# Chemical118/TREW

Hardware: AMD Instinct MI355X
Metric: Gbases/s scanned (short 5 32, 150 bp reads) (higher is better)
Workload: dtype u32

## Files before the change

include/trew_hip.h:

```cpp
#ifndef TREW_HIP_H
#define TREW_HIP_H

#include <stddef.h>
#include <stdint.h>

#ifdef __cplusplus
extern "C" {
#endif

#define TREW_HIP_ABI_VERSION 4

enum {
    TREW_MODE_SHORT = 0,
    TREW_MODE_PAIR = 1,
    TREW_MODE_LONG = 2,
    TREW_MODE_SEGMENT = 3
};

enum {
    TREW_TABLE_FORWARD_HIGH = 0,
    TREW_TABLE_FORWARD_LOW = 1,
    TREW_TABLE_BACKWARD_HIGH = 2,
    TREW_TABLE_BACKWARD_LOW = 3,
    TREW_TABLE_BOTH_HIGH = 4,
    TREW_TABLE_BOTH_LOW = 5,
    TREW_NUM_TABLES = 6
};

enum {
    TREW_FLAG_NO_FILTER = 1,
    TREW_FLAG_DEBUG_NO_EMIT = 2,
    TREW_FLAG_DEBUG_NO_KLOOP = 4,
    TREW_FLAG_DEBUG_POISON_LDS = 32,
    TREW_FLAG_DEBUG_WIDE_NO_WAIT = 128,
    TREW_FLAG_NO_TIMING = 64,
    TREW_FLAG_COMPAT_G1 = 512,
    TREW_FLAG_DEBUG_NO_JOINT = 2048,
    TREW_FLAG_DEBUG_NO_UNI_DRAIN = 4096,
    TREW_FLAG_DEBUG_NO_GROUP = 1024,
    TREW_FLAG_DEBUG_ANNOT_GENERAL = 8192,
    TREW_FLAG_TRACK_PRESSURE = 256
};

typedef struct {
    int32_t min_mer;
    int32_t max_mer;
    double low_baseline;
    double high_baseline;
    int32_t slice_length;
    int32_t mode;
    int32_t device;
    int32_t n_slots;
    uint64_t max_batch_words;
    uint64_t max_batch_reads;
    uint32_t table_log2_slots;
    uint32_t flags;
    uint64_t max_batch_ascii_bytes;
} trew_hip_params;

typedef struct {
    const uint32_t *words;
    uint64_t n_words;
    const uint32_t *offsets;
    const uint32_t *lengths;
    uint32_t uniform_length;
    uint32_t uniform_stride;
    uint64_t n_reads;
    int32_t on_device;
    int32_t max_length;
} trew_hip_batch;

// ... 106 lines not shown
```

trew_amd/__init__.py:

```python
from . import capi
from .capi import (
    FLAG_NO_FILTER,
    FLAG_DEBUG_ANNOT_GENERAL,
    FLAG_DEBUG_POISON_LDS,
    FLAG_NO_TIMING,
    FLAG_TRACK_PRESSURE,
    FLAG_COMPAT_G1,
    FLAG_DEBUG_NO_GROUP,
    FLAG_DEBUG_NO_JOINT,
    FLAG_DEBUG_NO_UNI_DRAIN,
    FLAG_DEBUG_WIDE_NO_WAIT,
    MODE_LONG,
    MODE_PAIR,
    MODE_SEGMENT,
    MODE_SHORT,
    TABLE_NAMES,
    TrewHip,
    TrewHipError,
    annotate,
    k_mer_check,
    pack_reads,
)
```

trew_amd/capi.py:

```python
from __future__ import annotations

import ctypes as C
import os

import numpy as np

_HERE = os.path.dirname(os.path.abspath(__file__))
LIB_PATH = os.environ.get("TREW_HIP_LIB") or os.path.join(_HERE, "lib", "libtrew_hip.so")

MODE_SHORT, MODE_PAIR, MODE_LONG, MODE_SEGMENT = 0, 1, 2, 3
FLAG_NO_FILTER = 1
FLAG_DEBUG_POISON_LDS = 32
FLAG_NO_TIMING = 64
FLAG_COMPAT_G1 = 512
FLAG_TRACK_PRESSURE = 256
FLAG_DEBUG_NO_JOINT = 2048
FLAG_DEBUG_NO_UNI_DRAIN = 4096
FLAG_DEBUG_NO_GROUP = 1024
FLAG_DEBUG_ANNOT_GENERAL = 8192
FLAG_DEBUG_WIDE_NO_WAIT = 128
TABLE_NAMES = ("forward_high", "forward_low", "backward_high", "backward_low", "both_high", "both_low")

EXPORTED_SYMBOLS = (
    "trew_hip_init", "trew_hip_destroy", "trew_hip_last_error", "trew_hip_submit", "trew_hip_wait",
    "trew_hip_collect", "trew_hip_reset_tables", "trew_hip_add_rows", "trew_hip_segment_results",
    "trew_hip_filter_masks", "trew_hip_last_timing", "trew_pack_words", "trew_pack_reads",
    "trew_synth_short_ascii", "trew_synth_short_device", "trew_synth_pair_ascii", "trew_synth_pair_device",
    "trew_hip_malloc", "trew_hip_free", "trew_hip_memcpy_h2d", "trew_hip_memcpy_d2h", "trew_hip_abi_version",
    "trew_pack_pairs", "trew_hip_host_alloc", "trew_hip_host_free", "trew_hip_device_count",
    "trew_synth_long_lengths", "trew_synth_long_ascii", "trew_synth_long_device",
    "trew_hip_collect_device", "trew_hip_add_rows_device", "trew_hip_merge", "trew_hip_table_pressure",
    "trew_hip_add_gathered_device", "trew_hip_collect_slice_device", "trew_hip_debug_counters", "trew_hip_debug_worklist", "trew_hip_submit_ascii", "trew_hip_pack_ascii",
    "trew_motif_parse", "trew_hip_annotate", "trew_hip_annotate_results", "trew_annotate_host",
)
DEBUG_COUNTERS = ("strict_rerun", "windows_fallback", "wide_spin_timeout", "inserted", "inserted_wide", "group_punt", "group_routed", "group_target")


class Params(C.Structure):
    _fields_ = [
        ("min_mer", C.c_int32), ("max_mer", C.c_int32),
        ("low_baseline", C.c_double), ("high_baseline", C.c_double),
        ("slice_length", C.c_int32), ("mode", C.c_int32), ("device", C.c_int32), ("n_slots", C.c_int32),
        ("max_batch_words", C.c_uint64), ("max_batch_reads", C.c_uint64),
        ("table_log2_slots", C.c_uint32), ("flags", C.c_uint32),
        ("max_batch_ascii_bytes", C.c_uint64),
    ]


class Batch(C.Structure):
    _fields_ = [
# ... 473 lines not shown
```

trew_amd/csrc/kernels/decide_group.inc:

```

#define TREW_REGION_LIST(X) \
    X(chunk) X(stage) X(group_setup) X(bounds) X(group) X(dg_loop) X(dg_pick) X(dg_eval) X(er_gaps) X(er_runs) X(er_canon) X(er_merge) X(er_max) \
    X(dg_decision) X(dg_end) X(routing) X(records) X(target) X(target_rows) X(target_eval) X(target_emit) X(fallback)
#define TREW_REGION_ENUM(n) kRegion_##n,
enum { TREW_REGION_LIST(TREW_REGION_ENUM) kRegionCount };
#ifdef TREW_REGION_COUNTS
__device__ unsigned long long g_region[64];
#define TREW_MARK(n)                                                                   \
    do {                                                                               \
        asm volatile("; MARK " #n);                                                    \
        if (lane_id() == 0) atomicAdd(&g_region[kRegion_##n], 1ull);                   \
    } while (0)
#else
#define TREW_MARK(n) asm volatile("; MARK " #n)
#endif
__device__ __forceinline__ void lds_sync() {
    __builtin_amdgcn_fence(__ATOMIC_RELEASE, "wavefront");
    __builtin_amdgcn_wave_barrier();
    __builtin_amdgcn_fence(__ATOMIC_ACQUIRE, "wavefront");
}
#define TREW_DPP(v, ctrl) ((u32) __builtin_amdgcn_update_dpp(0, (int) (v), (ctrl), 0xf, 0xf, false))
__device__ __forceinline__ u32 swap16(u32 v) { return (u32) __builtin_amdgcn_ds_swizzle((int) v, 0x401F); }
template <int G = 16>
__device__ __forceinline__ u32 row_or(u32 v) {
// ... 242 lines not shown
    }
}

template <int NW>
struct RowSeg {
    u32 lo[NW], hi[NW], v1[NW], P1[NW], P2[NW], P3[NW];
    u32 has_n;
};
template <int NW, int G = 16>
__device__ __forceinline__ void row_load(ExactSmem sm, int L, RowSeg<NW> &r) {
    const u32 g = lane_id() / (u32) G;
    const u32 *prep = sm_group(sm) + kGroupBnd + g * (6u * NW);
    u32 anyn = 0;
#pragma unroll
    for (int w = 0; w < NW; w++) {
        r.lo[w] = prep[0 * NW + w];
        r.hi[w] = prep[1 * NW + w];
        r.v1[w] = prep[2 * NW + w];
        r.P1[w] = prep[3 * NW + w];
        r.P2[w] = prep[4 * NW + w];
        r.P3[w] = prep[5 * NW + w];
        const int bits = L - 32 * w;
        const u32 lm = bits >= 32 ? 0xffffffffu : (bits <= 0 ? 0u : ((1u << bits) - 1u));
        anyn |= ~r.v1[w] & lm;
    }
    r.has_n = anyn != 0u ? 1u : 0u;
}

template <int NW, bool SMALLK>
__device__ __forceinline__ u32 shr_k_word(const u32 (&x)[NW], int w, u32 k) {
    if (SMALLK) return alignbit(w + 1 < NW ? x[w + 1 < NW ? w + 1 : 0] : 0u, x[w], k);
    return shr_var_word<NW>(x, w, k);
}
template <int NW, bool SMALLK = false>
__device__ __forceinline__ u32 bound_at_k(const RowSeg<NW> &r, int L, int k, int gmax, const DevParams &P) {
    const u32 ku = (u32) k;
    u32 V[NW];
    if (r.has_n == 0u) {
        const int wbits = L - k + 1;
#pragma unroll
        for (int w = 0; w < NW; w++) {
            const int bits = wbits - 32 * w;
            V[w] = bits >= 32 ? 0xffffffffu : (bits <= 0 ? 0u : ((1u << bits) - 1u));
        }
    } else {
        u32 A[NW];
#pragma unroll
        for (int w = 0; w < NW; w++) {
            V[w] = 0xffffffffu;
            A[w] = r.v1[w];
        }
        u32 off = 0;
#pragma unroll
        for (int b = 1; b <= 32; b <<= 1) {
            if (b > 1) {
                u32 T2[NW];
#pragma unroll
                for (int w = 0; w < NW; w++) T2[w] = A[w] & shr_var_word<NW>(A, w, (u32) (b / 2));
#pragma unroll
                for (int w = 0; w < NW; w++) A[w] = T2[w];
            }
            const bool take = (ku & (u32) b) != 0;
#pragma unroll
            for (int w = 0; w < NW; w++) {
                const u32 sh = shr_var_word<NW>(A, w, off);
                V[w] &= take ? sh : 0xffffffffu;
            }
            off += take ? (u32) b : 0u;
        }
    }
    u32 c000 = 0, c001 = 0, c010 = 0, c011 = 0, c100 = 0, c101 = 0, c110 = 0, c111 = 0, count = 0, links = 0;
    u32 Ew[NW];
#pragma unroll
    for (int w = 0; w < NW; w++) {
        const u32 F1 = r.P1[w] ^ shr_k_word<NW, SMALLK>(r.P1, w, ku), F2 = r.P2[w] ^ shr_k_word<NW, SMALLK>(r.P2, w, ku);
        const u32 F3 = r.P3[w] ^ shr_k_word<NW, SMALLK>(r.P3, w, ku);
        const u32 v = V[w];
        Ew[w] = ~((r.lo[w] ^ shr_k_word<NW, SMALLK>(r.lo, w, ku)) | (r.hi[w] ^ shr_k_word<NW, SMALLK>(r.hi, w, ku)));
        const u32 a1 = v & F1, a0 = v ^ a1;
        const u32 a11 = a1 & F2, a10 = a1 ^ a11, a01 = a0 & F2, a00 = a0 ^ a01;
        const u32 b111 = a11 & F3, b101 = a10 & F3, b011 = a01 & F3, b001 = a00 & F3;
        count += __popc(v);
        c111 += __popc(b111);
        c110 += __popc(a11 ^ b111);
        c101 += __popc(b101);
        c100 += __popc(a10 ^ b101);
        c011 += __popc(b011);
        c010 += __popc(a01 ^ b011);
        c001 += __popc(b001);
        c000 += __popc(a00 ^ b001);
    }
#pragma unroll
    for (int w = 0; w < NW; w++) {
        const u32 vn = w + 1 < NW ? V[w + 1 < NW ? w + 1 : 0] : 0u;
        links += __popc(V[w] & Ew[w] & alignbit(vn, V[w], 1u));
    }
    const u32 m8 = max(max(max(c000, c001), max(c010, c011)), max(max(c100, c101), max(c110, c111)));
    const u32 runs = count - links < 127u ? count - links : 127u;
    const double dm = (double) m8, dc = (double) count;
    const double tl = P.low * dc, th = P.high * dc;
    u32 pass_lo = dm > tl ? 1u : 0u, pass_hi = dm > th ? 1u : 0u;
    const bool amb = fabs(dm - tl) <= 1e-9 || fabs(dm - th) <= 1e-9;
    if (__any(amb)) {
        const double ub = count ? dm / dc : 0.0;
        pass_lo = ub >= P.low ? 1u : 0u;
        pass_hi = ub >= P.high ? 1u : 0u;
    }
    const bool inr = k <= gmax && count != 0u;
    return inr ? (m8 | (count << 10) | (runs << 20) | (pass_lo << 27) | (pass_hi << 28) | (r.has_n << 29)) : (r.has_n << 29);
}

template <typename WT>
struct GroupOut {
    u32 kk;
    WT sh, sl;
    u32 saved;
    WT kept_canon;
    u32 kept_cnt;
    bool punt;
};

template <int NW, typename WT, bool WANT_SEQ, int G = 16>
__device__ __forceinline__ GroupOut<WT> decide_group(ExactSmem sm, const DevParams &P, const RowSeg<NW> &rs, u32 bnd0, u32 bnd1, u32 range, const Segment &sg,
                                                     bool valid) {
    static_assert(sizeof(WT) == 8, "k <= 32: the k range must fit a 32-bit index mask");
    PH_T0(t_ph);
    const u32 lane = lane_id(), j = lane & (u32) (G - 1), gbase = lane & (u32) (64 - G);
    const u32 *grp = sm_group(sm);
    const u32 (&lo)[NW] = rs.lo;
    const u32 (&hi)[NW] = rs.hi;
    const int L = (int) sg.len;
    const u32 s0 = range_base(sm, range) + sg.start;
    const u32 has_n = rs.has_n;
    GroupOut<WT> o;
    o.kk = 0;
    o.sh = o.sl = 0;
    o.saved = 0;
    o.kept_canon = 0;
    o.kept_cnt = 0;
    u32 todo = 0;
    {
        const u32 a = (u32) (sg.kmin - P.min_mer) & 31u, b = (u32) (sg.kmax - P.min_mer);
// ... 149 lines not shown
    const u32 lane = lane_id();
#if defined(TREW_AB_SKIP) && TREW_AB_SKIP >= 5
    return;
#endif
    TREW_MARK(stage);
    PH_T0(t_stage);
    stage_two(sm, rdA, rdB, haveB);
    PH_ADD(PH_STAGE, t_stage);
#if defined(TREW_AB_SKIP) && TREW_AB_SKIP >= 4
    return;
#endif
    TREW_MARK(group_setup);
    const u32 g = lane >> 4, j = lane & 15u;
    const bool second = g >= 2u;
    const u32 is_right = g & 1u;
    ReadRef rd;
    rd.w = second ? rdB.w : rdA.w;
    rd.len = second ? rdB.len : rdA.len;
    rd.nw = second ? rdB.nw : rdA.nw;
    const Segment sg = get_segment(TREW_MODE_SHORT, (int) is_right, rd.len, 0, P.min_mer, P.max_mer, P.slice_len);
    const bool rowvalid = sg.valid && (!second || haveB);
    TREW_MARK(bounds);
    PH_T0(t_bounds);
    lds_sync();
    row_prepare<NW>(sm, rd, sg, rowvalid);
    lds_sync();
    RowSeg<NW> rs;
    row_load<NW>(sm, (int) sg.len, rs);
    u32 bnd0;
    if (P.min_mer + 15 < 32)
        bnd0 = rowvalid ? bound_at_k<NW, true>(rs, (int) sg.len, P.min_mer + (int) j, P.max_mer, P) : 0u;
    else
        bnd0 = rowvalid ? bound_at_k<NW, false>(rs, (int) sg.len, P.min_mer + (int) j, P.max_mer, P) : 0u;
    const u32 bnd1 = rowvalid ? bound_at_k<NW>(rs, (int) sg.len, P.min_mer + 16 + (int) j, P.max_mer, P) : 0u;
#if defined(TREW_AB_SKIP) && TREW_AB_SKIP >= 3
    asm volatile("" ::"v"(bnd0), "v"(bnd1));
    return;
#endif
    PH_ADD(PH_BOUNDS, t_bounds);
    TREW_MARK(group);
    const GroupOut<WT> o = decide_group<NW, WT, false>(sm, P, rs, bnd0, bnd1, second ? 1u : 0u, sg, rowvalid);
#if defined(TREW_AB_SKIP) && TREW_AB_SKIP >= 2
    asm volatile("" ::"v"(o.kk), "v"(o.saved), "v"(o.kept_cnt), "v"((u32) o.kept_canon), "v"((u32) (o.kept_canon >> 32)), "v"((u32) o.punt));
    return;
#endif
    TREW_MARK(routing);
    PH_T0(t_route);
    const u32 mine = rowvalid ? (o.kk | (o.punt ? 1u << 16 : 0u)) : 0u;
    const u32 other = lane_gather(mine, lane ^ 16u);
    const u32 kkL = is_right ? other : mine, kkR = is_right ? mine : other;
    const u32 lkh = kkL & 255u, lkl = (kkL >> 8) & 255u, rkh = kkR & 255u, rkl = (kkR >> 8) & 255u;
    const u32 left_found = (lkh | lkl) != 0u ? 1u : 0u;
    const u32 tgt_h = left_found & (lkh == rkh ? 1u : 0u) & (lkh != 0u ? 1u : 0u);
    const u32 tgt_l = left_found & (lkl == rkl ? 1u : 0u) & (lkl != 0u ? 1u : 0u);
    const u32 myk = o.saved & 255u, items = (o.saved >> 8) & 255u;
    u32 need_old = ((kkL | kkR) >> 16) & 1u;
    u32 rec_mask = 0;
    {
        const u32 kh = is_right ? rkh : lkh, kl = is_right ? rkl : lkl;
        const u32 rec_h = (kh != 0u ? 1u : 0u) & (is_right ? ((left_found ^ 1u) | (lkh == 0u ? 1u : 0u)) : (tgt_h ^ 1u));
        const u32 rec_l = (kl != 0u ? 1u : 0u) & (is_right ? ((left_found ^ 1u) | (lkl == 0u ? 1u : 0u)) : (tgt_l ^ 1u));
        const u32 th = is_right ? (1u << TREW_TABLE_BACKWARD_HIGH) : (1u << TREW_TABLE_FORWARD_HIGH);
        const u32 tl = is_right ? (1u << TREW_TABLE_BACKWARD_LOW) : (1u << TREW_TABLE_FORWARD_LOW);
        rec_mask = ((rec_h & (kh == myk ? 1u : 0u)) ? th : 0u) | ((rec_l & (kl == myk ? 1u : 0u)) ? tl : 0u);
        need_old |= (rec_h & (kh != myk ? 1u : 0u)) | (rec_l & (kl != myk ? 1u : 0u));
    }
    need_old |= tgt_h & tgt_l & (lkh != lkl ? 1u : 0u);
// ... 129 lines not shown
```

trew_amd/csrc/kernels/driver_pair.inc:

```

__device__ __forceinline__ u32 pack_intent(int slot, int k, int b, int temp) {
    return (u32) slot | ((u32) k << 3) | ((u32) b << 10) | ((u32) temp << 11) | (1u << 12);
}

__device__ __forceinline__ u32 dest(int temp, int b, int table) { return (1u << table) << (8 * (2 * temp + b)); }

template <typename WT>
__device__ __forceinline__ WT dir_seq(int i, int k, WT seq, bool is_for) {
    if ((i <= 2) == is_for) return seq;
    return min_rotation<WT>(revcomp(seq, k), k);
}

template <int NW, typename WT>
__device__ void run_pair(ExactSmem sm, const DevParams &P, TableRef T, u32 unit_in, const ReadRef r0_in, const ReadRef r1_in) {
    constexpr bool UB = NW > 0;
    constexpr int NWB = NW > 0 ? NW : 1;
    const u64 unit = rfl(unit_in);
    const ReadRef r0 = uni(r0_in), r1 = uni(r1_in);
    PH_CNT(PH_N_READS, 1);
    const int n1 = (int) r0.len, n2 = (int) r1.len;
    const int n = n1 < n2 ? n1 : n2;
    if (2 * P.min_mer > n) return;
    const bool in_lds = 3u * r0.nw <= sm.rawwords && 3u * r1.nw <= sm.rawwords;
    PH_T0(t_st);
    if (in_lds) {
        stage_two(sm, r0, r1, true);
    } else {
        stage_bases(sm, r0, 0, (u32) n1, 0);
        stage_bases(sm, r1, 0, (u32) n2, 1);
    }
    PH_ADD(PH_PAIR_STAGE, t_st);
    u32 my_intent = 0;
    u32 n_int = 0;
    const u32 lane = lane_id();
    auto seg_of = [&](int slot) { return get_segment(TREW_MODE_PAIR, slot, (u32) n1, (u32) n2, P.min_mer, P.max_mer, P.slice_len); };
    u32 dc_k = 0, dc_have = 0, dc_saved = 0;
    WT dc_sh = 0, dc_sl = 0;
    LaneMasks<NWB> mp;
    int mp_pair = -1;
    if constexpr (UB && sizeof(WT) == 8 && (NW == 3 || NW == 5)) {
        if (4 * P.min_mer <= n && P.max_mer - P.min_mer < 32 && !(P.flags & TREW_FLAG_DEBUG_NO_GROUP) && in_lds) {
            const u32 g = lane >> 4, j = lane & 15u;
            const Segment sg = get_segment(TREW_MODE_PAIR, (int) g, (u32) n1, (u32) n2, P.min_mer, P.max_mer, P.slice_len);
            ReadRef rd;
            rd.w = sg.mate ? r1.w : r0.w;
            rd.len = sg.mate ? r1.len : r0.len;
            rd.nw = sg.mate ? r1.nw : r0.nw;
            __syncthreads();
            row_prepare<NWB>(sm, rd, sg, true);
            __syncthreads();
            RowSeg<NWB> rs;
            row_load<NWB>(sm, (int) sg.len, rs);
            const u32 bnd0 = bound_at_k<NWB>(rs, (int) sg.len, P.min_mer + (int) j, P.max_mer, P);
            const u32 bnd1 = bound_at_k<NWB>(rs, (int) sg.len, P.min_mer + 16 + (int) j, P.max_mer, P);
            const GroupOut<WT> o = decide_group<NWB, WT, true>(sm, P, rs, bnd0, bnd1, sg.mate, sg, true);
            if (!(P.flags & TREW_FLAG_COMPAT_G1)) {
                const u32 kk0 = lane_gather(o.kk, 0u);
                const WT sh0 = lane_gather(o.sh, 0u);
                const u32 kh = o.kk & 255u, kl = (o.kk >> 8) & 255u, sk = o.saved & 255u;
                const WT fh = strand_flip<WT>(o.sh, (int) (kh ? kh : 1u));
                bool okr = !o.punt && o.kk == kk0 && kh != 0u && kh == kl && sk == kh && o.sh == o.sl;
                if (okr) okr = (g < 2u ? o.sh : fh) == sh0;
                if (__ballot(okr) == ~0ull) {
                    const DevTable Tv = load_table(T);
                    const u32 cnt = j < ((o.saved >> 8) & 255u) ? o.kept_cnt : 0u;
                    const bool is_x = cnt != 0u && o.kept_canon == o.sh;
                    const u32 cx = row_max<16>(is_x ? cnt : 0u);
                    const u32 total = (u32) __builtin_amdgcn_readlane((int) cx, 0) + (u32) __builtin_amdgcn_readlane((int) cx, 16) +
                                      (u32) __builtin_amdgcn_readlane((int) cx, 32) + (u32) __builtin_amdgcn_readlane((int) cx, 48);
                    const u32 add = is_x ? (g == 0u ? total : 0u) : cnt;
                    if (add != 0u) {
                        const WT w = strand_canon<WT>(o.kept_canon, (int) kh);
                        cached_add(sm, Tv, TREW_TABLE_BOTH_HIGH, (int) kh, w, add);
                        cached_add(sm, Tv, TREW_TABLE_BOTH_LOW, (int) kh, w, add);
                    }
                    PH_CNT(PH_N_RECORD, 1);
                    return;
                }
                if (4 * P.max_mer <= n && __ballot(o.punt) == 0ull) {
                    const WT fl = strand_flip<WT>(o.sl, (int) (kl ? kl : 1u));
                    u32 recF[2], recB[2];
                    int si[2];
                    u32 tk[2][4];
                    WT ts[2][4], tf[2][4];
#pragma unroll
                    for (int s = 0; s < 4; s++) {
                        const u32 c = (u32) __builtin_amdgcn_readlane((int) o.kk, 16 * s);
// ... 372 lines not shown
```

trew_amd/csrc/kernels/exact_core.inc:

```

struct ExactSmem {
    u32 lds;
    u32 cap, rawwords;
    u32 s0;
    u32 rs, rnw;
    const u32 *rw;
};
__host__ __device__ inline u32 exact_rangewords(u32 cap) { return cap / 32 + 2; }

constexpr u32 kCacheSlots = 128;
constexpr u32 kRawReads = 8;
constexpr u32 kIntentWords = 64;
constexpr u32 kGroupBnd = 0, kGroupMult = 128, kGroupRes = 160, kGroupWords = 192;
constexpr u32 kGroupPairIndex = kGroupRes + 31;
__host__ __device__ inline u32 exact_lds_precache(u32 cap, u32 rawwords) {
    const u32 b = 2 * exact_rangewords(cap) * 8 + 2 * (cap / 64 + 2) * 8 + 2 * exact_rangewords(cap) * 4 + kRawReads * rawwords * 4 + 2 * cap * 2 + (kIntentWords + kGroupWords) * 4;
    return (b + 15u) & ~15u;
}
__host__ __device__ inline u32 exact_lds_fixed(u32 cap, u32 rawwords) {
    return exact_lds_precache(cap, rawwords) + kCacheSlots * 16u;
}
constexpr u32 kSaveItems = 16, kSaveSlots = 6;
__host__ __device__ inline u32 exact_lds_bytes(u32 cap, u32 rawwords, u32 wordbytes) {
    return exact_lds_fixed(cap, rawwords) + cap * wordbytes + 16 + kSaveSlots * kSaveItems * (wordbytes + 2u);
// ... 630 lines not shown
            const u32 per = (u32) __builtin_popcount(table_mask);
            const u64 have = __ballot(c != 0);
            u32 at = 0;
            if (lane == 0 && have) at = atomicAdd(&counters[0], per * (u32) __builtin_popcountll(have));
            at = rfl(at) + per * (u32) __builtin_popcountll(have & ((1ull << lane) - 1ull));
            if (c) {
                for (u32 tm = table_mask; tm; tm &= tm - 1, at++) {
                    if (at < log_cap) {
                        trew_hip_row r;
                        r.k = k;
                        r.table = __ffs((int) tm) - 1;
                        r.word_lo = (u64) w;
                        r.word_hi = pair;
                        r.count = c;
                        log[at] = r;
                    } else {
                        atomicAdd(&T.overflow[kDiagG1Drop], 1u);
                    }
                }
            }
        }
        if (c) {
            if (negate) {
                for (u32 tm = table_mask; tm; tm &= tm - 1) table_add(T, __ffs((int) tm) - 1, k, w, 0ull - (u64) c);
            } else {
                for (u32 tm = table_mask; tm; tm &= tm - 1) cached_add(sm, T, __ffs((int) tm) - 1, k, w, c);
            }
        }
    }
    PH_ADD(PH_EMIT, t_ph);
}

template <int NW>
__device__ __forceinline__ u32 shr_var_word(const u32 (&x)[NW], int j, u32 off) {
    const bool big = off >= 32u;
    const u32 x0 = x[j], x1 = j + 1 < NW ? x[j + 1 < NW ? j + 1 : 0] : 0u, x2 = j + 2 < NW ? x[j + 2 < NW ? j + 2 : 0] : 0u;
    return alignbit(big ? x2 : x1, big ? x1 : x0, off & 31u);
}

template <int NW>
struct LaneMasks {
    u32 V[NW];
    u32 E[NW];
    double ub;
    u32 runs;
    u32 m8, cnt;
    bool has_n;
};

template <int NW>
__device__ __forceinline__ void lane_bounds_at(const ReadRef &rd, u32 s, int L, int k, int gmax, LaneMasks<NW> &out);
template <int NW>
__device__ __forceinline__ void lane_bounds(const ReadRef &rd, u32 s, int L, int gmin, int gmax, LaneMasks<NW> &out) {
    lane_bounds_at<NW>(rd, s, L, gmin + (int) lane_id(), gmax, out);
}
template <int NW>
__device__ __forceinline__ void lane_bounds_pair(const ReadRef &rd, u32 sA, int LA, u32 sB, int LB, int gmin, int gmax, LaneMasks<NW> &out) {
    const bool hiHalf = lane_id() >= 32u;
    lane_bounds_at<NW>(rd, hiHalf ? sB : sA, hiHalf ? LB : LA, gmin + (int) (lane_id() & 31u), gmax, out);
}
template <int NW>
__device__ __forceinline__ void lane_bounds_at(const ReadRef &rd, u32 s, int L, int k, int gmax, LaneMasks<NW> &out) {
    PH_T0(t_ph);
    u32 lo[NW], hi[NW], nm[NW];
    load_planes<NW>(rd, s, lo, hi, nm);
    u32 v1[NW], P1[NW], P2[NW], P3[NW];
    {
        u32 f1[NW], f2[NW], f3[NW];
#pragma unroll
        for (int j = 0; j < NW; j++) {
            int bits = L - 32 * j;
            u32 lm = bits >= 32 ? 0xffffffffu : (bits <= 0 ? 0u : ((1u << bits) - 1u));
            v1[j] = ~nm[j] & lm;
// ... 560 lines not shown
```

trew_amd/csrc/kernels/helpers.inc:

```

__device__ u32 g_fallback[kFallbackWords];
__device__ __forceinline__ void count_fallback(int which) {
    if ((threadIdx.x & 63u) == 0) atomicAdd(&g_fallback[which], 1u);
}
__device__ __forceinline__ u32 alignbit(u32 hi, u32 lo, u32 sh) {
    return __builtin_amdgcn_alignbit(hi, lo, sh);
}
__device__ __forceinline__ u32 lane_id() { return threadIdx.x & 63u; }
__device__ __forceinline__ u32 bcnt_acc(u32 x, u32 acc) {
    u32 d;
    asm("v_bcnt_u32_b32 %0, %1, %2" : "=v"(d) : "v"(x), "v"(acc));
    return d;
}
struct MultiplesTable {
    u64 v[65];
    constexpr MultiplesTable() : v() {
        for (int k = 1; k <= 64; k++) {
            u64 m = 0;
            for (int j = k; j <= 64; j += k) m |= 1ull << (j - 1);
            v[k] = m;
        }
    }
};
__constant__ MultiplesTable kMultiples = MultiplesTable();
__device__ __forceinline__ u64 load_multiples(int k) { return kMultiples.v[k & 127 ? (k <= 64 ? k : 0) : 0]; }
__device__ __forceinline__ u32 rfl(u32 v) { return __builtin_amdgcn_readfirstlane(v); }
__device__ __forceinline__ u64 rfl64(u64 v) {
    u32 lo = __builtin_amdgcn_readfirstlane((u32) v);
    u32 hi = __builtin_amdgcn_readfirstlane((u32) (v >> 32));
    return ((u64) hi << 32) | lo;
}

__device__ __forceinline__ int rfl_i(int v) { return __builtin_amdgcn_readfirstlane(v); }
template <typename Tp>
__device__ __forceinline__ Tp *rfl_ptr(Tp *p) {
    return (Tp *) rfl64((u64) p);
}
__device__ __forceinline__ double rfl_f64(double v) {
    return __hiloint2double(__builtin_amdgcn_readfirstlane(__double2hiint(v)), __builtin_amdgcn_readfirstlane(__double2loint(v)));
}

// ... 97 lines not shown
```

trew_amd/csrc/kernels/prefilter.inc:

```


template <int NW>
__device__ __forceinline__ void prefix_parity(const u32 (&f)[NW], u32 (&P)[NW]) {
    u32 carry = 0, prev_top = 0;
#pragma unroll
    for (int j = 0; j < NW; j++) {
        u32 x = f[j];
        x ^= x << 1;
        x ^= x << 2;
        x ^= x << 4;
        x ^= x << 8;
        x ^= x << 16;
        x ^= carry;
        P[j] = (x << 1) | prev_top;
        prev_top = x >> 31;
        carry = 0u - prev_top;
    }
}

template <>
__device__ __forceinline__ void prefix_parity<3>(const u32 (&f)[3], u32 (&P)[3]) {
    u64 x = ((u64) f[1] << 32) | f[0];
    x ^= x << 1;
    x ^= x << 2;
// ... 562 lines not shown
    u32 c001 = 0, c010 = 0, c011 = 0, c100 = 0, c101 = 0, c110 = 0, c111 = 0;
#pragma unroll
    for (int j = 0; j < N; j++) {
        const u32 a11 = F1[j] & F2[j], a10 = F1[j] & ~F2[j], a01 = ~F1[j] & F2[j], a00 = V[j] & ~(F1[j] | F2[j]);
        const u32 b111 = a11 & F3[j], b101 = a10 & F3[j], b011 = a01 & F3[j], b001 = a00 & F3[j];
        c111 += __popc(b111);
        c110 += __popc(a11 ^ b111);
        c101 += __popc(b101);
        c100 += __popc(a10 ^ b101);
        c011 += __popc(b011);
        c010 += __popc(a01 ^ b011);
        c001 += __popc(b001);
    }
    const u32 c000 = count - c001 - c010 - c011 - c100 - c101 - c110 - c111;
    const u32 m8 = max(max(max(c000, c001), max(c010, c011)), max(max(c100, c101), max(c110, c111)));
    return (int) m8 >= ithr;
}

__device__ __forceinline__ bool drain_uni_applies(const DevParams &P, u32 UL, int gmax_run) {
    const int n_halves = P.mode == TREW_MODE_PAIR ? 4 : (P.mode == TREW_MODE_SHORT ? 2 : 0);
    if (n_halves == 0) return false;
    for (int slot = n_halves; slot < mode_slots(P.mode); slot++)
        if (get_segment(P.mode, slot, UL, UL, P.min_mer, P.max_mer, P.slice_len).valid) return false;
    for (int p = 0; p < n_halves; p += 2) {
        const Segment a = get_segment(P.mode, p, UL, UL, P.min_mer, P.max_mer, P.slice_len);
        const Segment b = get_segment(P.mode, p + 1, UL, UL, P.min_mer, P.max_mer, P.slice_len);
        const int la = (int) a.len, lb = (int) b.len, lmin = la < lb ? la : lb, lmax = la < lb ? lb : la;
        const int khi = a.kmax < gmax_run ? a.kmax : gmax_run;
        if (!(a.valid && b.valid && a.kmin == b.kmin && a.kmax == b.kmax && lmax <= 95 && lmax - lmin <= 1 && a.kmin >= 1 && khi <= lmin)) return false;
    }
    return true;
}

__device__ __forceinline__ bool filter_deferred_uni(const DevParams &P, const DevBatch &B, u64 unit, bool active, int gmax_run,
                                                    const int4 *cnt_thr) {
    const u32 UL = B.uniform_length;
    ReadRef rd[2];
    rd[0].w = B.words;
    rd[0].len = 0;
    rd[0].nw = 0;
    rd[1] = rd[0];
    if (active) {
        if (P.mode == TREW_MODE_PAIR) {
            rd[0] = get_read(B, 2 * unit);
            rd[1] = get_read(B, 2 * unit + 1);
        } else {
            rd[0] = get_read(B, unit);
        }
    }
    const u64 actm = __ballot(active);
    u64 flag = 0;
    const int n_halves = P.mode == TREW_MODE_PAIR ? 4 : 2;
    for (int p = 0; p < n_halves && flag != actm; p += 2) {
        const Segment sA = get_segment(P.mode, p, UL, UL, P.min_mer, P.max_mer, P.slice_len);
        const Segment sB = get_segment(P.mode, p + 1, UL, UL, P.min_mer, P.max_mer, P.slice_len);
        const int LA = rfl_i((int) sA.len), LB = rfl_i((int) sB.len), Lmax = LA < LB ? LB : LA;
        const int klo = rfl_i(sA.kmin > P.min_mer ? sA.kmin : P.min_mer), khi = rfl_i(sA.kmax < gmax_run ? sA.kmax : gmax_run);
        DrainHalf A, Bh;
        {
            u32 lo[3], hi[3], nm[3];
            load_planes<3>(sA.mate ? rd[1] : rd[0], sA.start, lo, hi, nm);
            drain_half_init(lo, hi, nm, LA, active, A);
            load_planes<3>(sB.mate ? rd[1] : rd[0], sB.start, lo, hi, nm);
            drain_half_init(lo, hi, nm, LB, active, Bh);
        }
        for (int t = 1; t < klo; t++) {
            drain_v_step3(A.V);
            drain_v_step3(Bh.V);
        }
        int k = klo;
        {
            const int b = khi < Lmax - 64 ? khi : Lmax - 64;
            auto half3 = [&](const DrainHalf &h, u32 bs) __attribute__((always_inline)) -> u64 {
                const u32 cnt = bcnt_acc(h.V[2], bcnt_acc(h.V[1], __popc(h.V[0])));
                const int4 th = cnt_thr[cnt];
                u32 F1[3], F2[3];
#pragma unroll
                for (int j = 0; j < 3; j++) {
                    F1[j] = xor_and(h.P1[j], alignbit(j < 2 ? h.P1[j < 2 ? j + 1 : 0] : 0u, h.P1[j], bs), h.V[j]);
                    F2[j] = xor_and(h.P2[j], alignbit(j < 2 ? h.P2[j < 2 ? j + 1 : 0] : 0u, h.P2[j], bs), h.V[j]);
                }
                const u64 p4 = __ballot(drain_signs<3>(F1, F2, th) >= 0);
                u64 p8 = 0;
                if (p4 & ~flag) {
                    u32 F3[3];
#pragma unroll
                    for (int j = 0; j < 3; j++) F3[j] = h.P3[j] ^ alignbit(j < 2 ? h.P3[j < 2 ? j + 1 : 0] : 0u, h.P3[j], bs);
                    p8 = __ballot(drain_pass8<3>(F1, F2, F3, h.V, cnt, th.w));
                }
                return p8;
            };
            for (; k <= b && flag != actm; k++) {
                flag |= half3(A, (u32) k);
                flag |= half3(Bh, (u32) k);
                drain_v_step3(A.V);
                drain_v_step3(Bh.V);
            }
        }
        if (k <= khi && flag != actm) {
            const int oA = LA > 63 ? LA - 63 : 0, oB = LB > 63 ? LB - 63 : 0;
            const u64 QA1 = container64(A.P1, oA), QA2 = container64(A.P2, oA), QB1 = container64(Bh.P1, oB), QB2 = container64(Bh.P2, oB);
            u64 VA = ((u64) A.V[1] << 32) | A.V[0], VB = ((u64) Bh.V[1] << 32) | Bh.V[0];
            auto half2 = [&](const DrainHalf &h, u64 Q1, u64 Q2, u64 V, int s) __attribute__((always_inline)) -> u64 {
                const u32 v0 = (u32) V, v1 = (u32) (V >> 32);
                const u32 cnt = bcnt_acc(v1, __popc(v0));
                const int4 th = cnt_thr[cnt];
                const u32 sh = (u32) (k - s);
                const u64 S1 = Q1 >> sh, S2 = Q2 >> sh;
                const u32 F1[2] = {xor_and(h.P1[0], (u32) S1, v0), xor_and(h.P1[1], (u32) (S1 >> 32), v1)};
                const u32 F2[2] = {xor_and(h.P2[0], (u32) S2, v0), xor_and(h.P2[1], (u32) (S2 >> 32), v1)};
                const u64 p4 = __ballot(drain_signs<2>(F1, F2, th) >= 0);
                u64 p8 = 0;
                if (p4 & ~flag) {
                    const u64 S3 = container64(h.P3, s) >> sh;
                    const u32 F3[2] = {h.P3[0] ^ (u32) S3, h.P3[1] ^ (u32) (S3 >> 32)};
                    const u32 Vw[2] = {v0, v1};
                    p8 = __ballot(drain_pass8<2>(F1, F2, F3, Vw, cnt, th.w));
                }
                return p8;
            };
            for (; k <= khi && flag != actm; k++) {
                flag |= half2(A, QA1, QA2, VA, oA);
                flag |= half2(Bh, QB1, QB2, VB, oB);
                VA &= VA >> 1;
                VB &= VB >> 1;
            }
        }
    }
    return (flag >> lane_id()) & 1ull;
}

constexpr u32 kFilterThreads = TREW_FILTER_THREADS;
constexpr u32 kStage = kFilterThreads == 256 ? 1024 : 192;
constexpr u32 kDefer = 2 * kFilterThreads;

template <int NW>
#ifndef TREW_FILTER3_WAVES
#define TREW_FILTER3_WAVES 6
#endif
#ifndef TREW_FILTER5_WAVES
#define TREW_FILTER5_WAVES 6
#endif
__global__ __launch_bounds__(kFilterThreads, (NW <= 3 ? TREW_FILTER3_WAVES : (NW == 5 ? TREW_FILTER5_WAVES : 1))) void filter_kernel(DevParams P, DevBatch B, u32 *wl, u32 *wl_count, u32 wl_cap,
                                                                u64 *dbg_masks, int dbg_slots, int max_seg, u32 *diag,
                                                                const int2 *__restrict__ thr_tab) {
#ifdef TREW_AB_FILTER_PRIO
// ... 67 lines not shown
                    if (ok) {
                        load_planes<NW>(r, sg.start, lo, hi, nm);
                    } else {
#pragma unroll
                        for (int j = 0; j < NW; j++) {
                            lo[j] = hi[j] = 0;
                            nm[j] = 0xffffffffu;
                        }
                    }
                    u64 m;
                    if (P.flags & TREW_FLAG_NO_FILTER)
                        m = all_k_mask(sg.kmin, sg.kmax);
                    else
                        m = filter_segment<NW>(lo, hi, nm, ok ? (int) sg.len : 0, sg.kmin, sg.kmax, P.min_mer, gmax_run, max_seg, P.lowf);
                    mask = ok ? m : 0ull;
                }
                if (active && sg.valid && sg.len > (u32) (32 * NW - 1)) mask = all_k_mask(sg.kmin, sg.kmax);
                any |= mask;
                if (dbg_masks && active && slot < dbg_slots) dbg_masks[unit * (u64) dbg_slots + slot] = mask;
            }
        }
        return any;
    };

    __shared__ u32 defer[kDefer];
    __shared__ unsigned char defer_kind[kDefer];
    __shared__ u32 wm_tab[34];
    if (threadIdx.x < 34) wm_tab[threadIdx.x] = threadIdx.x < 32 ? 0xffffffffu >> threadIdx.x : 0u;
    __shared__ int4 cnt_thr[kCntThr];
    for (u32 i = threadIdx.x; i < (u32) kCntThr; i += blockDim.x) cnt_thr[i] = count_thresholds((int) i, P.lowf);
    const u32 UL = B.uniform_length;
    const bool uni = NW <= 5 && UL != 0 && thr_tab != nullptr && P.mode != TREW_MODE_LONG && !(P.flags & TREW_FLAG_NO_FILTER);
    const bool uni_drain = NW == 3 && uni && !dbg_masks && !(P.flags & TREW_FLAG_DEBUG_NO_UNI_DRAIN) && drain_uni_applies(P, UL, gmax_run);
    if (threadIdx.x == 0) defer_n = 0;
    __syncthreads();
    __shared__ u32 next_chunk[2];
    constexpr u32 kChunkShards = 8;
    const u32 my_shard = blockIdx.x & (kChunkShards - 1u);
    auto shard_ctr = [&](u32 sh) __attribute__((always_inline)) { return wl_count + 32u + 32u * sh + kChunkCounterWord; };
    u64 chunk = blockIdx.x;
    u32 round = 0;
    for (;;) {
        const bool more = chunk * kFilterThreads < B.n_units;
        if (more) {
            const u64 unit = chunk * kFilterThreads + threadIdx.x;
            const bool active = unit < B.n_units;
            u32 nxt = 0;
#ifndef TREW_AB_STATIC_CHUNKS
            if (threadIdx.x == 0) nxt = gridDim.x + kChunkShards * atomicAdd(shard_ctr(my_shard), 1u) + my_shard;
#else
            nxt = (u32) chunk + gridDim.x;
#endif
            u64 any = 0;
            bool dfr = active, dfr_n = false;
            if constexpr (NW <= 5) {
                if (uni) {
                    ReadRef rd[2];
                    rd[0].w = B.words;
                    rd[0].len = 0;
                    rd[0].nw = 0;
                    rd[1] = rd[0];
                    if (active) {
                        if (P.mode == TREW_MODE_PAIR) {
                            rd[0] = get_read(B, 2 * unit);
                            rd[1] = get_read(B, 2 * unit + 1);
                        } else {
// ... 73 lines not shown
                    if (dfr) {
                        const u32 at = sb + (u32) __popcll(bal & ((1ull << lane) - 1ull));
                        defer[at] = (u32) unit;
                        defer_kind[at] = dfr_n ? 1 : 0;
                    }
                }
            }
            if (threadIdx.x == 0) next_chunk[round & 1u] = nxt;
            append(active && !dfr && any != 0, (u32) unit);
            chunk = next_chunk[round & 1u];
#ifndef TREW_AB_STATIC_CHUNKS
            if (chunk * kFilterThreads >= B.n_units) {
                __syncthreads();
                if (threadIdx.x == 0) {
                    u64 c = chunk;
                    for (u32 att = 1; att < kChunkShards && c * kFilterThreads >= B.n_units; att++) {
                        const u32 sh = (my_shard + att) & (kChunkShards - 1u);
                        c = (u64) gridDim.x + (u64) kChunkShards * atomicAdd(shard_ctr(sh), 1u) + sh;
                    }
                    next_chunk[round & 1u] = (u32) (c < 0xffffffffull ? c : 0xffffffffull);
                }
                __syncthreads();
                chunk = next_chunk[round & 1u];
                __syncthreads();
            }
#endif
            round++;
        }
        const u32 dn = defer_seen;
        if (dn >= kFilterThreads || (!more && dn > 0u)) {
            const u32 take = dn < kFilterThreads ? dn : kFilterThreads;
            const u32 at = dn - take;
            const bool active2 = threadIdx.x < take;
            const u32 unit2 = active2 ? defer[at + threadIdx.x] : 0u;
            const bool n2 = active2 && defer_kind[at + threadIdx.x] != 0;
            __syncthreads();
            if (threadIdx.x == 0) defer_n = at;
#ifndef TREW_AB_SKIP_DRAIN
            const u64 any2 = uni_drain ? (u64) filter_deferred_uni(P, B, unit2, active2, gmax_run, cnt_thr) : general(unit2, active2);
#else
            u64 any2 = 0;
            u32 keep = unit2;
            asm volatile("" : "+v"(keep), "+v"(any2));
            (void) keep;
#endif
            append(active2 && any2 != 0 && !n2, unit2);
            append(active2 && any2 != 0 && n2, unit2);
        } else if (!more) {
            break;
        }
    }
    flush();
}
```

Baseline: 1996.

## Partition deferred drain by N-content and add fast N-free halves path

Before the uniform drain, the deferred units are reordered within the block so that units containing N and N-free units sit in separate waves. Waves with no N units can then take a new path that screens k values with cheaper halves-threshold candidates and runs the full 8-class check only on survivors. Separately, the upper-k bound computation for NW=3 uses only two window words when no lane needs more, and c000 is derived from the count rather than popcounted. The reordering costs extra LDS traffic and two block barriers per drain round, and the new path adds code size and register pressure.

```diff
diff --git a/include/trew_hip.h b/include/trew_hip.h
--- a/include/trew_hip.h
+++ b/include/trew_hip.h
@@ -37,6 +37,7 @@
     TREW_FLAG_COMPAT_G1 = 512,
     TREW_FLAG_DEBUG_NO_JOINT = 2048,
     TREW_FLAG_DEBUG_NO_UNI_DRAIN = 4096,
+    TREW_FLAG_DEBUG_NO_DRAIN_SPLIT = 16384,
     TREW_FLAG_DEBUG_NO_GROUP = 1024,
     TREW_FLAG_DEBUG_ANNOT_GENERAL = 8192,
     TREW_FLAG_TRACK_PRESSURE = 256
diff --git a/trew_amd/__init__.py b/trew_amd/__init__.py
--- a/trew_amd/__init__.py
+++ b/trew_amd/__init__.py
@@ -9,6 +9,7 @@
     FLAG_DEBUG_NO_GROUP,
     FLAG_DEBUG_NO_JOINT,
     FLAG_DEBUG_NO_UNI_DRAIN,
+    FLAG_DEBUG_NO_DRAIN_SPLIT,
     FLAG_DEBUG_WIDE_NO_WAIT,
     MODE_LONG,
     MODE_PAIR,
diff --git a/trew_amd/capi.py b/trew_amd/capi.py
--- a/trew_amd/capi.py
+++ b/trew_amd/capi.py
@@ -16,6 +16,7 @@
 FLAG_TRACK_PRESSURE = 256
 FLAG_DEBUG_NO_JOINT = 2048
 FLAG_DEBUG_NO_UNI_DRAIN = 4096
+FLAG_DEBUG_NO_DRAIN_SPLIT = 16384
 FLAG_DEBUG_NO_GROUP = 1024
 FLAG_DEBUG_ANNOT_GENERAL = 8192
 FLAG_DEBUG_WIDE_NO_WAIT = 128
diff --git a/trew_amd/csrc/kernels/decide_group.inc b/trew_amd/csrc/kernels/decide_group.inc
--- a/trew_amd/csrc/kernels/decide_group.inc
+++ b/trew_amd/csrc/kernels/decide_group.inc
@@ -298,24 +298,25 @@
     if (SMALLK) return alignbit(w + 1 < NW ? x[w + 1 < NW ? w + 1 : 0] : 0u, x[w], k);
     return shr_var_word<NW>(x, w, k);
 }
-template <int NW, bool SMALLK = false>
+template <int NW, bool SMALLK = false, int NWW = NW>
 __device__ __forceinline__ u32 bound_at_k(const RowSeg<NW> &r, int L, int k, int gmax, const DevParams &P) {
+    static_assert(NWW >= 1 && NWW <= NW, "window words are a prefix of the segment's words");
     const u32 ku = (u32) k;
-    u32 V[NW];
+    u32 V[NWW], count;
     if (r.has_n == 0u) {
         const int wbits = L - k + 1;
 #pragma unroll
-        for (int w = 0; w < NW; w++) {
+        for (int w = 0; w < NWW; w++) {
             const int bits = wbits - 32 * w;
             V[w] = bits >= 32 ? 0xffffffffu : (bits <= 0 ? 0u : ((1u << bits) - 1u));
         }
+        count = wbits > 0 ? (u32) wbits : 0u;
     } else {
         u32 A[NW];
 #pragma unroll
-        for (int w = 0; w < NW; w++) {
-            V[w] = 0xffffffffu;
-            A[w] = r.v1[w];
-        }
+        for (int w = 0; w < NW; w++) A[w] = r.v1[w];
+#pragma unroll
+        for (int w = 0; w < NWW; w++) V[w] = 0xffffffffu;
         u32 off = 0;
 #pragma unroll
         for (int b = 1; b <= 32; b <<= 1) {
@@ -328,17 +329,20 @@
             }
             const bool take = (ku & (u32) b) != 0;
 #pragma unroll
-            for (int w = 0; w < NW; w++) {
+            for (int w = 0; w < NWW; w++) {
                 const u32 sh = shr_var_word<NW>(A, w, off);
                 V[w] &= take ? sh : 0xffffffffu;
             }
             off += take ? (u32) b : 0u;
         }
-    }
-    u32 c000 = 0, c001 = 0, c010 = 0, c011 = 0, c100 = 0, c101 = 0, c110 = 0, c111 = 0, count = 0, links = 0;
-    u32 Ew[NW];
-#pragma unroll
-    for (int w = 0; w < NW; w++) {
+        count = 0;
+#pragma unroll
+        for (int w = 0; w < NWW; w++) count += __popc(V[w]);
+    }
+    u32 c001 = 0, c010 = 0, c011 = 0, c100 = 0, c101 = 0, c110 = 0, c111 = 0, links = 0;
+    u32 Ew[NWW];
+#pragma unroll
+    for (int w = 0; w < NWW; w++) {
         const u32 F1 = r.P1[w] ^ shr_k_word<NW, SMALLK>(r.P1, w, ku), F2 = r.P2[w] ^ shr_k_word<NW, SMALLK>(r.P2, w, ku);
         const u32 F3 = r.P3[w] ^ shr_k_word<NW, SMALLK>(r.P3, w, ku);
         const u32 v = V[w];
@@ -346,7 +350,6 @@
         const u32 a1 = v & F1, a0 = v ^ a1;
         const u32 a11 = a1 & F2, a10 = a1 ^ a11, a01 = a0 & F2, a00 = a0 ^ a01;
         const u32 b111 = a11 & F3, b101 = a10 & F3, b011 = a01 & F3, b001 = a00 & F3;
-        count += __popc(v);
         c111 += __popc(b111);
         c110 += __popc(a11 ^ b111);
         c101 += __popc(b101);
@@ -354,11 +357,11 @@
         c011 += __popc(b011);
         c010 += __popc(a01 ^ b011);
         c001 += __popc(b001);
-        c000 += __popc(a00 ^ b001);
-    }
-#pragma unroll
-    for (int w = 0; w < NW; w++) {
-        const u32 vn = w + 1 < NW ? V[w + 1 < NW ? w + 1 : 0] : 0u;
+    }
+    const u32 c000 = count - c001 - c010 - c011 - c100 - c101 - c110 - c111;
+#pragma unroll
+    for (int w = 0; w < NWW; w++) {
+        const u32 vn = w + 1 < NWW ? V[w + 1 < NWW ? w + 1 : 0] : 0u;
         links += __popc(V[w] & Ew[w] & alignbit(vn, V[w], 1u));
     }
     const u32 m8 = max(max(max(c000, c001), max(c010, c011)), max(max(c100, c101), max(c110, c111)));
@@ -374,6 +377,17 @@
     }
     const bool inr = k <= gmax && count != 0u;
     return inr ? (m8 | (count << 10) | (runs << 20) | (pass_lo << 27) | (pass_hi << 28) | (r.has_n << 29)) : (r.has_n << 29);
+}
+
+#ifndef TREW_AB_BOUND_WORDS
+#define TREW_AB_BOUND_WORDS 1
+#endif
+template <int NW>
+__device__ __forceinline__ u32 bound_at_k_upper(const RowSeg<NW> &r, int L, int k, int gmax, const DevParams &P, bool valid) {
+    if constexpr (NW == 3 && TREW_AB_BOUND_WORDS) {
+        if (!__any(valid && L - (P.min_mer + 16) + 1 > 64)) return valid ? bound_at_k<NW, false, 2>(r, L, k, gmax, P) : 0u;
+    }
+    return valid ? bound_at_k<NW>(r, L, k, gmax, P) : 0u;
 }
 
 template <typename WT>
@@ -589,7 +603,7 @@
         bnd0 = rowvalid ? bound_at_k<NW, true>(rs, (int) sg.len, P.min_mer + (int) j, P.max_mer, P) : 0u;
     else
         bnd0 = rowvalid ? bound_at_k<NW, false>(rs, (int) sg.len, P.min_mer + (int) j, P.max_mer, P) : 0u;
-    const u32 bnd1 = rowvalid ? bound_at_k<NW>(rs, (int) sg.len, P.min_mer + 16 + (int) j, P.max_mer, P) : 0u;
+    const u32 bnd1 = bound_at_k_upper<NW>(rs, (int) sg.len, P.min_mer + 16 + (int) j, P.max_mer, P, rowvalid);
 #if defined(TREW_AB_SKIP) && TREW_AB_SKIP >= 3
     asm volatile("" ::"v"(bnd0), "v"(bnd1));
     return;
diff --git a/trew_amd/csrc/kernels/driver_pair.inc b/trew_amd/csrc/kernels/driver_pair.inc
--- a/trew_amd/csrc/kernels/driver_pair.inc
+++ b/trew_amd/csrc/kernels/driver_pair.inc
@@ -52,7 +52,7 @@
             RowSeg<NWB> rs;
             row_load<NWB>(sm, (int) sg.len, rs);
             const u32 bnd0 = bound_at_k<NWB>(rs, (int) sg.len, P.min_mer + (int) j, P.max_mer, P);
-            const u32 bnd1 = bound_at_k<NWB>(rs, (int) sg.len, P.min_mer + 16 + (int) j, P.max_mer, P);
+            const u32 bnd1 = bound_at_k_upper<NWB>(rs, (int) sg.len, P.min_mer + 16 + (int) j, P.max_mer, P, true);
             const GroupOut<WT> o = decide_group<NWB, WT, true>(sm, P, rs, bnd0, bnd1, sg.mate, sg, true);
             if (!(P.flags & TREW_FLAG_COMPAT_G1)) {
                 const u32 kk0 = lane_gather(o.kk, 0u);
diff --git a/trew_amd/csrc/kernels/exact_core.inc b/trew_amd/csrc/kernels/exact_core.inc
--- a/trew_amd/csrc/kernels/exact_core.inc
+++ b/trew_amd/csrc/kernels/exact_core.inc
@@ -686,13 +686,6 @@
 }
 
 template <int NW>
-__device__ __forceinline__ u32 shr_var_word(const u32 (&x)[NW], int j, u32 off) {
-    const bool big = off >= 32u;
-    const u32 x0 = x[j], x1 = j + 1 < NW ? x[j + 1 < NW ? j + 1 : 0] : 0u, x2 = j + 2 < NW ? x[j + 2 < NW ? j + 2 : 0] : 0u;
-    return alignbit(big ? x2 : x1, big ? x1 : x0, off & 31u);
-}
-
-template <int NW>
 struct LaneMasks {
     u32 V[NW];
     u32 E[NW];
diff --git a/trew_amd/csrc/kernels/helpers.inc b/trew_amd/csrc/kernels/helpers.inc
--- a/trew_amd/csrc/kernels/helpers.inc
+++ b/trew_amd/csrc/kernels/helpers.inc
@@ -7,6 +7,12 @@
     return __builtin_amdgcn_alignbit(hi, lo, sh);
 }
 __device__ __forceinline__ u32 lane_id() { return threadIdx.x & 63u; }
+template <int NW>
+__device__ __forceinline__ u32 shr_var_word(const u32 (&x)[NW], int j, u32 off) {
+    const bool big = off >= 32u;
+    const u32 x0 = x[j], x1 = j + 1 < NW ? x[j + 1 < NW ? j + 1 : 0] : 0u, x2 = j + 2 < NW ? x[j + 2 < NW ? j + 2 : 0] : 0u;
+    return alignbit(big ? x2 : x1, big ? x1 : x0, off & 31u);
+}
 __device__ __forceinline__ u32 bcnt_acc(u32 x, u32 acc) {
     u32 d;
     asm("v_bcnt_u32_b32 %0, %1, %2" : "=v"(d) : "v"(x), "v"(acc));
diff --git a/trew_amd/csrc/kernels/prefilter.inc b/trew_amd/csrc/kernels/prefilter.inc
--- a/trew_amd/csrc/kernels/prefilter.inc
+++ b/trew_amd/csrc/kernels/prefilter.inc
@@ -618,8 +618,92 @@
     return true;
 }
 
-__device__ __forceinline__ bool filter_deferred_uni(const DevParams &P, const DevBatch &B, u64 unit, bool active, int gmax_run,
-                                                    const int4 *cnt_thr) {
+struct HalvesFail {
+    u32 a, b;
+};
+__device__ __forceinline__ u32 half_nopass(u32 x, u32 t) { return __builtin_amdgcn_bitop3_b32(x, t, t, 0x30); }
+__device__ __forceinline__ HalvesFail halves_candidates_uni(const HalvesP &A, const HalvesP &Bh, int L, int klo, int khi, const int4 *__restrict__ thr_row,
+                                                            const u32 *wm_tab) {
+    HalvesFail f;
+    f.a = f.b = 0xffffffffu;
+    int k = klo;
+    const int4 *tp = thr_row + (klo - 1);
+    {
+        int b = L - 64;
+        b = b > khi ? khi : b;
+        for (; k <= b; k++, tp++) {
+            const int4 t = load_thr4(tp);
+            const u32 bs = (u32) k;
+            u32 xA, tA, xB, tB;
+            halves_signs(A.P1[0] ^ alignbit(A.P1[1], A.P1[0], bs), A.P2[0] ^ alignbit(A.P2[1], A.P2[0], bs), A.P1[1] ^ alignbit(A.P1[2], A.P1[1], bs),
+                         A.P2[1] ^ alignbit(A.P2[2], A.P2[1], bs), t.x, t.y, t.z, xA, tA);
+            halves_signs(Bh.P1[0] ^ alignbit(Bh.P1[1], Bh.P1[0], bs), Bh.P2[0] ^ alignbit(Bh.P2[1], Bh.P2[0], bs), Bh.P1[1] ^ alignbit(Bh.P1[2], Bh.P1[1], bs),
+                         Bh.P2[1] ^ alignbit(Bh.P2[2], Bh.P2[1], bs), t.x, t.y, t.z, xB, tB);
+            f.a = alignbit(f.a, half_nopass(xA, tA), 31u);
+            f.b = alignbit(f.b, half_nopass(xB, tB), 31u);
+        }
+    }
+    if (k <= khi) {
+        const int s = L > 63 ? L - 63 : 0;
+        const u64 QA1 = container64(A.P1, s), QA2 = container64(A.P2, s), QB1 = container64(Bh.P1, s), QB2 = container64(Bh.P2, s);
+        for (; k <= khi; k++, tp++) {
+            const int4 t = load_thr4(tp);
+            const u32 shk = (u32) (k - s);
+            const u32 wmk = wm_tab[63 - (L - k)];
+            const u64 SA1 = QA1 >> shk, SA2 = QA2 >> shk, SB1 = QB1 >> shk, SB2 = QB2 >> shk;
+            const u32 gA1 = xor_and(A.P1[1], (u32) (SA1 >> 32), wmk), gA2 = xor_and(A.P2[1], (u32) (SA2 >> 32), wmk);
+            const u32 gB1 = xor_and(Bh.P1[1], (u32) (SB1 >> 32), wmk), gB2 = xor_and(Bh.P2[1], (u32) (SB2 >> 32), wmk);
+            u32 xA, tA, xB, tB;
+            halves_signs(A.P1[0] ^ (u32) SA1, A.P2[0] ^ (u32) SA2, gA1, gA2, t.x, t.y, t.z, xA, tA);
+            halves_signs(Bh.P1[0] ^ (u32) SB1, Bh.P2[0] ^ (u32) SB2, gB1, gB2, t.x, t.y, t.z, xB, tB);
+            f.a = alignbit(f.a, half_nopass(xA, tA), 31u);
+            f.b = alignbit(f.b, half_nopass(xB, tB), 31u);
+        }
+    }
+    return f;
+}
+__device__ __forceinline__ u64 half_verdicts8(const u32 (&lo)[3], const u32 (&hi)[3], int L, int khi, u32 cand, const int4 *cnt_thr) {
+    u32 P1[3], P2[3], P3[3];
+    {
+        u32 f1[3], f2[3], f3[3];
+#pragma unroll
+        for (int j = 0; j < 3; j++) {
+            const int bits = L - 32 * j;
+            const u32 lm = bits >= 32 ? 0xffffffffu : (bits <= 0 ? 0u : ((1u << bits) - 1u));
+            f1[j] = lo[j] & lm;
+            f2[j] = hi[j] & lm;
+            f3[j] = f1[j] & f2[j];
+        }
+        prefix_parity<3>(f1, P1);
+        prefix_parity<3>(f2, P2);
+        prefix_parity<3>(f3, P3);
+    }
+    u64 flag = 0;
+    while (__any(cand != 0u)) {
+        const bool have = cand != 0u;
+        const u32 i = have ? (u32) __builtin_ctz(cand) : 0u;
+        cand &= cand - 1u;
+        const u32 k = (u32) khi - i;
+        const u32 W = have ? (u32) L - k + 1u : 0u;
+        u32 V[3], F1[3], F2[3], F3[3];
+#pragma unroll
+        for (int j = 0; j < 3; j++) {
+            const int bits = (int) W - 32 * j;
+            V[j] = bits >= 32 ? 0xffffffffu : (bits <= 0 ? 0u : ((1u << bits) - 1u));
+            F1[j] = xor_and(P1[j], shr_var_word<3>(P1, j, k), V[j]);
+            F2[j] = xor_and(P2[j], shr_var_word<3>(P2, j, k), V[j]);
+            F3[j] = P3[j] ^ shr_var_word<3>(P3, j, k);
+        }
+        const bool p8 = drain_pass8<3>(F1, F2, F3, V, W, cnt_thr[W].w);
+        const u64 hit = __ballot(p8);
+        flag |= hit;
+        cand = p8 ? 0u : cand;
+    }
+    return flag;
+}
+
+__device__ __forceinline__ bool filter_deferred_uni(const DevParams &P, const DevBatch &B, u64 unit, bool active, bool has_n, bool nfree_ok, int gmax_run,
+                                                    const int4 *cnt_thr, const int2 *__restrict__ thr_tab, const u32 *wm_tab) {
     const u32 UL = B.uniform_length;
     ReadRef rd[2];
     rd[0].w = B.words;
@@ -642,6 +726,25 @@
         const Segment sB = get_segment(P.mode, p + 1, UL, UL, P.min_mer, P.max_mer, P.slice_len);
         const int LA = rfl_i((int) sA.len), LB = rfl_i((int) sB.len), Lmax = LA < LB ? LB : LA;
         const int klo = rfl_i(sA.kmin > P.min_mer ? sA.kmin : P.min_mer), khi = rfl_i(sA.kmax < gmax_run ? sA.kmax : gmax_run);
+        if (nfree_ok && __ballot(active && has_n) == 0ull && (LB == LA || LB == LA + 1) && klo <= khi && klo >= LA + 1 - kUniSubsetMax && khi <= LA - 32 &&
+            klo <= 31 && khi - klo <= 31) {
+            u32 loA[3], hiA[3], loB[3], hiB[3], nm[3];
+            load_planes<3>(sA.mate ? rd[1] : rd[0], sA.start, loA, hiA, nm);
+            load_planes<3>(sB.mate ? rd[1] : rd[0], sB.start, loB, hiB, nm);
+            HalvesFail f;
+            {
+                HalvesP hA, hB;
+                halves_prefix(loA, hiA, LA, hA);
+                halves_prefix(loB, hiB, LA, hB);
+                f = halves_candidates_uni(hA, hB, LA, klo, khi, joint_thresholds(thr_tab) + (LB != LA ? 2 + p / 2 : p / 2) * kThrRow, wm_tab);
+            }
+            const u32 kmask = 0xffffffffu >> (31 - (khi - klo));
+            const bool open = active && ((flag >> lane_id()) & 1ull) == 0ull;
+            flag |= half_verdicts8(loA, hiA, LA, khi, open ? ~f.a & kmask : 0u, cnt_thr);
+            const bool open2 = active && ((flag >> lane_id()) & 1ull) == 0ull;
+            flag |= half_verdicts8(loB, hiB, LB, khi, open2 ? ~f.b & kmask : 0u, cnt_thr);
+            continue;
+        }
         DrainHalf A, Bh;
         {
             u32 lo[3], hi[3], nm[3];
@@ -668,7 +771,12 @@
                 }
                 const u64 p4 = __ballot(drain_signs<3>(F1, F2, th) >= 0);
                 u64 p8 = 0;
+#ifdef TREW_AB_SKIP_DRAIN8
+                asm volatile("" ::"s"(p4));
+                if (false) {
+#else
                 if (p4 & ~flag) {
+#endif
                     u32 F3[3];
 #pragma unroll
                     for (int j = 0; j < 3; j++) F3[j] = h.P3[j] ^ alignbit(j < 2 ? h.P3[j < 2 ? j + 1 : 0] : 0u, h.P3[j], bs);
@@ -697,7 +805,12 @@
                 const u32 F2[2] = {xor_and(h.P2[0], (u32) S2, v0), xor_and(h.P2[1], (u32) (S2 >> 32), v1)};
                 const u64 p4 = __ballot(drain_signs<2>(F1, F2, th) >= 0);
                 u64 p8 = 0;
+#ifdef TREW_AB_SKIP_DRAIN8
+                asm volatile("" ::"s"(p4));
+                if (false) {
+#else
                 if (p4 & ~flag) {
+#endif
                     const u64 S3 = container64(h.P3, s) >> sh;
                     const u32 F3[2] = {h.P3[0] ^ (u32) S3, h.P3[1] ^ (u32) (S3 >> 32)};
                     const u32 Vw[2] = {v0, v1};
@@ -831,6 +944,9 @@
     const u32 UL = B.uniform_length;
     const bool uni = NW <= 5 && UL != 0 && thr_tab != nullptr && P.mode != TREW_MODE_LONG && !(P.flags & TREW_FLAG_NO_FILTER);
     const bool uni_drain = NW == 3 && uni && !dbg_masks && !(P.flags & TREW_FLAG_DEBUG_NO_UNI_DRAIN) && drain_uni_applies(P, UL, gmax_run);
+    constexpr u32 kFilterWaves = kFilterThreads / 64u;
+    __shared__ u32 split_cnt[2 * kFilterWaves];
+    const bool drain_split = uni_drain && kFilterWaves > 1u && !(P.flags & TREW_FLAG_DEBUG_NO_DRAIN_SPLIT);
     if (threadIdx.x == 0) defer_n = 0;
     __syncthreads();
     __shared__ u32 next_chunk[2];
@@ -970,12 +1086,39 @@
             const u32 take = dn < kFilterThreads ? dn : kFilterThreads;
             const u32 at = dn - take;
             const bool active2 = threadIdx.x < take;
-            const u32 unit2 = active2 ? defer[at + threadIdx.x] : 0u;
-            const bool n2 = active2 && defer_kind[at + threadIdx.x] != 0;
+            u32 unit2 = active2 ? defer[at + threadIdx.x] : 0u;
+            bool n2 = active2 && defer_kind[at + threadIdx.x] != 0;
             __syncthreads();
             if (threadIdx.x == 0) defer_n = at;
+            if (drain_split) {
+                const u32 wave = (u32) rfl_i((int) (threadIdx.x >> 6));
+                const u64 bn = __ballot(n2), bf = __ballot(active2 && !n2);
+                if (lane_id() == 0) {
+                    split_cnt[wave] = (u32) __popcll(bn);
+                    split_cnt[kFilterWaves + wave] = (u32) __popcll(bf);
+                }
+                __syncthreads();
+                u32 before_n = 0, before_f = 0, total_n = 0;
+#pragma unroll
+                for (u32 w = 0; w < kFilterWaves; w++) {
+                    const u32 cn = (u32) rfl_i((int) split_cnt[w]), cf = (u32) rfl_i((int) split_cnt[kFilterWaves + w]);
+                    total_n += cn;
+                    before_n += w < wave ? cn : 0u;
+                    before_f += w < wave ? cf : 0u;
+                }
+                const u32 below_n = __builtin_amdgcn_mbcnt_hi((u32) (bn >> 32), __builtin_amdgcn_mbcnt_lo((u32) bn, 0u));
+                const u32 below_f = __builtin_amdgcn_mbcnt_hi((u32) (bf >> 32), __builtin_amdgcn_mbcnt_lo((u32) bf, 0u));
+                const u32 pos = n2 ? before_n + below_n : total_n + before_f + below_f;
+                if (active2) {
+                    defer[at + pos] = unit2;
+                    defer_kind[at + pos] = n2 ? 1 : 0;
+                }
+                __syncthreads();
+                unit2 = active2 ? defer[at + threadIdx.x] : 0u;
+                n2 = active2 && defer_kind[at + threadIdx.x] != 0;
+            }
 #ifndef TREW_AB_SKIP_DRAIN
-            const u64 any2 = uni_drain ? (u64) filter_deferred_uni(P, B, unit2, active2, gmax_run, cnt_thr) : general(unit2, active2);
+            const u64 any2 = uni_drain ? (u64) filter_deferred_uni(P, B, unit2, active2, n2, drain_split, gmax_run, cnt_thr, thr_tab, wm_tab) : general(unit2, active2);
 #else
             u64 any2 = 0;
             u32 keep = unit2;
```

Result: no change. 2013 (median of 6 runs) (+0.9%).
